# SenseTime-FVG/OpenDWM

Measured on NVIDIA H100. Metric: CTSD-3.5 6view x 16f denoise-steps/sec, higher is better.
Workload: dtype fp16

## Files before the change

opendwm_b200/csrc/common.cuh:

```cuda
#pragma once

#include <cuda.h>
#include <cuda_runtime.h>
#include <cuda_bf16.h>
#include <cuda_fp16.h>
#include <cuda_fp8.h>
#include <stdint.h>
#include <stdio.h>

namespace dwm {

void set_last_error(const char* fmt, ...);

#define DWM_CHECK_CUDA(expr)                                                   \
  do {                                                                         \
    cudaError_t _e = (expr);                                                   \
    if (_e != cudaSuccess) {                                                   \
      ::dwm::set_last_error("%s failed: %s (%s:%d)", #expr,                    \
                            cudaGetErrorString(_e), __FILE__, __LINE__);       \
      return -2;                                                               \
    }                                                                          \
  } while (0)

#define DWM_REQUIRE(cond, ...)                                                 \
  do {                                                                         \
    if (!(cond)) {                                                             \
      ::dwm::set_last_error(__VA_ARGS__);                                      \
      return -1;                                                               \
    }                                                                          \
  } while (0)

int make_tmap_2d(CUtensorMap* map, const void* base, uint64_t rows, uint64_t cols,
                 uint64_t ld, uint32_t box_rows, uint32_t box_cols, int elem_bytes);

int make_tmap_nd(CUtensorMap* map, const void* base, int rank, const uint64_t* dims,
                 const uint64_t* strides_bytes, const uint32_t* box, int elem_bytes);

int sm_count();

inline bool is_aligned(const void* p, uintptr_t bytes) { return (reinterpret_cast<uintptr_t>(p) & (bytes - 1)) == 0; }

#ifdef __CUDACC__
__device__ __forceinline__ uint32_t smem_u32(const void* p) {
  return static_cast<uint32_t>(__cvta_generic_to_shared(p));
}

__device__ __forceinline__ bool elect_one() {
  uint32_t pred = 0;
  asm volatile(
      "{\n\t"
      ".reg .pred P;\n\t"
      "elect.sync _|P, 0xffffffff;\n\t"
      "selp.u32 %0, 1, 0, P;\n\t"
      "}\n"
      : "=r"(pred));
  return pred != 0;
}

__device__ __forceinline__ void mbar_init(uint64_t* bar, uint32_t count) {
  asm volatile("mbarrier.init.shared::cta.b64 [%0], %1;" ::"r"(smem_u32(bar)), "r"(count));
}
__device__ __forceinline__ void fence_barrier_init() {
  asm volatile("fence.mbarrier_init.release.cluster;" ::: "memory");
}
__device__ __forceinline__ void fence_proxy_async() {
  asm volatile("fence.proxy.async.shared::cta;" ::: "memory");
}
__device__ __forceinline__ void mbar_expect_tx(uint64_t* bar, uint32_t bytes) {
  asm volatile("mbarrier.arrive.expect_tx.shared::cta.b64 _, [%0], %1;" ::"r"(smem_u32(bar)),
               "r"(bytes)
               : "memory");
}
__device__ __forceinline__ void mbar_arrive(uint64_t* bar) {
  asm volatile("mbarrier.arrive.shared::cta.b64 _, [%0];" ::"r"(smem_u32(bar)) : "memory");
}
__device__ __forceinline__ bool mbar_try_wait(uint64_t* bar, uint32_t parity) {
  uint32_t ok;
  asm volatile(
      "{\n\t"
      ".reg .pred P;\n\t"
      "mbarrier.try_wait.parity.shared::cta.b64 P, [%1], %2;\n\t"
      "selp.u32 %0, 1, 0, P;\n\t"
      "}\n"
      : "=r"(ok)
      : "r"(smem_u32(bar)), "r"(parity)
      : "memory");
  return ok != 0;
}
__device__ __forceinline__ void mbar_wait(uint64_t* bar, uint32_t parity) {
#ifdef DWM_BOUNDED_WAIT
  for (uint32_t it = 0; it < (1u << 26); ++it) {
    if (mbar_try_wait(bar, parity)) return;
  }
  printf("dwm_b200: mbarrier wait timed out (block %d thread %d)\n", blockIdx.x, threadIdx.x);
  __trap();
#else
  while (!mbar_try_wait(bar, parity)) {
  }
#endif
}

__device__ __forceinline__ void tma_prefetch_desc(const CUtensorMap* m) {
  asm volatile("prefetch.tensormap [%0];" ::"l"(reinterpret_cast<uint64_t>(m)) : "memory");
}
__device__ __forceinline__ void tma_load_2d(const CUtensorMap* m, uint64_t* bar, void* smem,
                                            int32_t c0, int32_t c1, uint64_t cache_hint) {
  asm volatile(
      "cp.async.bulk.tensor.2d.shared::cluster.global.mbarrier::complete_tx::bytes.L2::cache_hint"
      " [%0], [%1, {%3, %4}], [%2], %5;"
      :
      : "r"(smem_u32(smem)), "l"(reinterpret_cast<uint64_t>(m)), "r"(smem_u32(bar)), "r"(c0),
        "r"(c1), "l"(cache_hint)
      : "memory");
}
constexpr uint64_t kEvictNormal = 0x1000000000000000ull;
constexpr uint64_t kEvictFirst = 0x12F0000000000000ull;
constexpr uint64_t kEvictLast = 0x14F0000000000000ull;
__device__ __forceinline__ void tma_prefetch_2d(const CUtensorMap* m, int32_t c0, int32_t c1) {
  asm volatile("cp.async.bulk.prefetch.tensor.2d.L2.global.tile [%0, {%1, %2}];" ::"l"(
                   reinterpret_cast<uint64_t>(m)),
               "r"(c0), "r"(c1)
               : "memory");
}
__device__ __forceinline__ void tma_prefetch_5d(const CUtensorMap* m, int c0, int c1, int c2, int c3, int c4) {
  asm volatile("cp.async.bulk.prefetch.tensor.5d.L2.global.tile [%0, {%1, %2, %3, %4, %5}];" ::"l"(
                   reinterpret_cast<uint64_t>(m)),
               "r"(c0), "r"(c1), "r"(c2), "r"(c3), "r"(c4)
               : "memory");
}
__device__ __forceinline__ void tma_load_5d(const CUtensorMap* m, uint64_t* bar, void* smem, int c0,
                                            int c1, int c2, int c3, int c4, uint64_t hint) {
  asm volatile(
      "cp.async.bulk.tensor.5d.shared::cluster.global.mbarrier::complete_tx::bytes.L2::cache_hint"
      " [%0], [%1, {%3, %4, %5, %6, %7}], [%2], %8;"
      :
      : "r"(smem_u32(smem)), "l"(reinterpret_cast<uint64_t>(m)), "r"(smem_u32(bar)), "r"(c0), "r"(c1),
        "r"(c2), "r"(c3), "r"(c4), "l"(hint)
      : "memory");
}

__device__ __forceinline__ uint32_t cluster_ctarank() {
  uint32_t r;
  asm volatile("mov.u32 %0, %%cluster_ctarank;" : "=r"(r));
  return r;
}
__device__ __forceinline__ void cluster_sync_all() {
  asm volatile("barrier.cluster.arrive.release.aligned;" ::: "memory");
  asm volatile("barrier.cluster.wait.acquire.aligned;" ::: "memory");
}
__device__ __forceinline__ uint32_t mapa_u32(uint32_t smem_addr, uint32_t rank) {
  uint32_t r;
  asm volatile("mapa.shared::cluster.u32 %0, %1, %2;" : "=r"(r) : "r"(smem_addr), "r"(rank));
  return r;
}
__device__ __forceinline__ void mbar_arrive_remote(uint32_t cluster_addr) {
  asm volatile("mbarrier.arrive.shared::cluster.b64 _, [%0];" ::"r"(cluster_addr) : "memory");
}
__device__ __forceinline__ void tma_load_2d_mc(const CUtensorMap* m, uint64_t* bar, void* smem, int32_t c0,
                                               int32_t c1, uint16_t mask, uint64_t cache_hint) {
  asm volatile(
      "cp.async.bulk.tensor.2d.shared::cluster.global.mbarrier::complete_tx::bytes.multicast::cluster"
      ".L2::cache_hint [%0], [%1, {%3, %4}], [%2], %5, %6;"
      :
      : "r"(smem_u32(smem)), "l"(reinterpret_cast<uint64_t>(m)), "r"(smem_u32(bar)), "r"(c0), "r"(c1),
        "h"(mask), "l"(cache_hint)
      : "memory");
}

__device__ __forceinline__ uint64_t gmma_desc_sw128(uint32_t smem_addr) {
  uint64_t d = 0;
  d |= static_cast<uint64_t>((smem_addr & 0x3FFFF) >> 4);
  d |= static_cast<uint64_t>(1) << 16;
  d |= static_cast<uint64_t>(1024 >> 4) << 32;
  d |= static_cast<uint64_t>(1) << 62;
  return d;
}
__device__ __forceinline__ void wgmma_fence() { asm volatile("wgmma.fence.sync.aligned;" ::: "memory"); }
__device__ __forceinline__ void wgmma_commit() { asm volatile("wgmma.commit_group.sync.aligned;" ::: "memory"); }
template <int N>
__device__ __forceinline__ void wgmma_wait() {
  asm volatile("wgmma.wait_group.sync.aligned %0;" ::"n"(N) : "memory");
}
template <int N>
__device__ __forceinline__ void fence_operands(float (&d)[N]) {
#pragma unroll
  for (int i = 0; i < N; ++i) asm volatile("" : "+f"(d[i])::"memory");
}
template <int R>
__device__ __forceinline__ void setmaxnreg_inc() { asm volatile("setmaxnreg.inc.sync.aligned.u32 %0;" ::"n"(R)); }
template <int R>
__device__ __forceinline__ void setmaxnreg_dec() { asm volatile("setmaxnreg.dec.sync.aligned.u32 %0;" ::"n"(R)); }

__device__ __forceinline__ float gelu_erf(float x) {
  return 0.5f * x * (1.0f + erff(x * 0.70710678118654752440f));
}
__device__ __forceinline__ float gelu_tanh(float x) {
  const float k2 = 2.0f * 0.7978845608028654f;
  const float u2 = k2 * (x + 0.044715f * x * x * x);
  return __fdividef(x, 1.0f + __expf(-u2));
}
__device__ __forceinline__ float silu(float x) { return x / (1.0f + __expf(-x)); }

template <typename T>
struct Cvt;
template <>
struct Cvt<__nv_bfloat16> {
  __device__ static __forceinline__ uint32_t pack2(float a, float b) {
    __nv_bfloat162 v = __floats2bfloat162_rn(a, b);
    return *reinterpret_cast<uint32_t*>(&v);
  }
  __device__ static __forceinline__ float2 unpack2(uint32_t u) {
    __nv_bfloat162 v = *reinterpret_cast<__nv_bfloat162*>(&u);
    return __bfloat1622float2(v);
  }
  __device__ static __forceinline__ float to_f(__nv_bfloat16 v) { return __bfloat162float(v); }
  __device__ static __forceinline__ __nv_bfloat16 from_f(float v) { return __float2bfloat16_rn(v); }
};
template <>
struct Cvt<__half> {
  __device__ static __forceinline__ uint32_t pack2(float a, float b) {
    __half2 v = __floats2half2_rn(a, b);
// ... 34 lines not shown
```

opendwm_b200/csrc/gemm.cu:

```cuda
#include <stdlib.h>
#include <string.h>

#include "gemm_epilogue.cuh"

namespace dwm {

constexpr int STAGES = 4;
constexpr int A_STAGE_BYTES = BM * BK * 2;

template <int NT>
struct GemmCfg {
  static constexpr int kBStageBytes = NT * BK * 2;
  static constexpr int kSmemBytes =
      STAGES * (A_STAGE_BYTES + kBStageBytes) + EPI_STAGE_BYTES + 1024  + 256 ;
};

template <typename TA, typename T, int EPI, int NT, int CL>
__global__ void __launch_bounds__(GEMM_THREADS, 1)
    gemm_wgmma_kernel(const __grid_constant__ CUtensorMap tmap_a,
                      const __grid_constant__ CUtensorMap tmap_b, int M, int N, int K,
                      EpiParams p) {
  constexpr int B_STAGE_BYTES = GemmCfg<NT>::kBStageBytes;
  constexpr int BKE = BK * 2 / static_cast<int>(sizeof(TA));
  extern __shared__ uint8_t smem_raw[];
  uint8_t* smem = smem_raw + ((1024u - (smem_u32(smem_raw) & 1023u)) & 1023u);
  uint8_t* smem_a = smem;
  uint8_t* smem_b = smem + STAGES * A_STAGE_BYTES;
  float* epi_stage = reinterpret_cast<float*>(smem + STAGES * (A_STAGE_BYTES + B_STAGE_BYTES));
  uint64_t* bars = reinterpret_cast<uint64_t*>(smem + STAGES * (A_STAGE_BYTES + B_STAGE_BYTES) + EPI_STAGE_BYTES);
  uint64_t* full_bar = bars;
  uint64_t* empty_bar = bars + STAGES;

  const int warp = threadIdx.x >> 5;
  const int lane = threadIdx.x & 31;
  const int wg = threadIdx.x >> 7;
  const uint32_t rank = CL == 2 ? cluster_ctarank() : 0u;

  const int m_blocks = (M + BM - 1) / BM;
  const int n_blocks = (N + NT - 1) / NT;
  const int k_blocks = (K + BKE - 1) / BKE;
  const int num_tiles = ((m_blocks + CL - 1) / CL) * n_blocks;
  const int first = static_cast<int>(blockIdx.x) / CL, step = static_cast<int>(gridDim.x) / CL;

  if (warp == 0 && lane == 0) {
    tma_prefetch_desc(&tmap_a);
    tma_prefetch_desc(&tmap_b);
    for (int s = 0; s < STAGES; ++s) {
      mbar_init(&full_bar[s], 1);
      mbar_init(&empty_bar[s], CL * EPI_WARPS);
    }
    fence_barrier_init();
  }
  if constexpr (CL == 2) cluster_sync_all(); else __syncthreads();

  if (wg == 0) {
    setmaxnreg_dec<PRODUCER_REGS>();
    if (warp == 0 && elect_one()) {
      int stage = 0;
      uint32_t phase = 0;
      for (int tile = first; tile < num_tiles; tile += step) {
        const int m_blk = (tile / n_blocks) * CL + static_cast<int>(rank);
        const int n_blk = tile % n_blocks;
        for (int kb = 0; kb < k_blocks; ++kb) {
          mbar_wait(&empty_bar[stage], phase ^ 1);
          mbar_expect_tx(&full_bar[stage], A_STAGE_BYTES + B_STAGE_BYTES);
          tma_load_2d(&tmap_a, &full_bar[stage], smem_a + stage * A_STAGE_BYTES, kb * BKE,
                      m_blk * BM, kEvictNormal);
          if constexpr (CL == 2) {
            tma_load_2d_mc(&tmap_b, &full_bar[stage], smem_b + stage * B_STAGE_BYTES + rank * (B_STAGE_BYTES / 2),
                           kb * BKE, n_blk * NT + static_cast<int>(rank) * (NT / 2), 0x3, kEvictLast);
          } else {
            tma_load_2d(&tmap_b, &full_bar[stage], smem_b + stage * B_STAGE_BYTES, kb * BKE,
                        n_blk * NT, kEvictLast);
          }
          if (++stage == STAGES) {
            stage = 0;
            phase ^= 1;
          }
        }
      }
    }
    __syncwarp();
  } else {
    setmaxnreg_inc<CONSUMER_REGS>();
    const int cw = wg - 1;
    const int wrow = cw * 64 + (warp & 3) * 16;
    float* stg = epi_stage + (warp - 4) * 512;
    int stage = 0;
    uint32_t phase = 0;
    for (int tile = first; tile < num_tiles; tile += step) {
      const int m_blk = (tile / n_blocks) * CL + static_cast<int>(rank);
      const int n_blk = tile % n_blocks;
      const int t = threadIdx.x & 127;
      prefetch_resid_tile<EPI, NT>(p, m_blk * BM + cw * 64 + (t >> 1), M, n_blk * NT, N, t & 1);
      float acc[NT / 2];
      wg_mainloop<TA, NT, CL>(acc, smem_a, A_STAGE_BYTES, cw * 64 * 128, smem_b, B_STAGE_BYTES, full_bar,
                              empty_bar, STAGES, k_blocks, stage, phase, lane, rank ^ 1u);
      if constexpr (sizeof(TA) == 1)
        dequant_frag<NT>(acc, p.a_scale, p.w_scale, m_blk * BM + wrow, M, n_blk * NT, N, lane);
      drain_tile<T, EPI, NT>(acc, stg, m_blk * BM, wrow, M, n_blk * NT, N, p, lane);
    }
  }
  if constexpr (CL == 2) cluster_sync_all();
}

int g_resid_tma = 1;

template <typename TA, typename T, int EPI, int NT, int CL>
static int launch_gemm(const dwm_linear_args* a, cudaStream_t stream) {
  constexpr int eb = static_cast<int>(sizeof(TA));
  CUtensorMap ta, tb;
  int rc = make_tmap_2d(&ta, a->A, a->M, a->K, a->lda, BM, BK * 2 / eb, eb);
  if (rc) return rc;
  rc = make_tmap_2d(&tb, a->W, a->N, a->K, a->ldw, NT / CL, BK * 2 / eb, eb);
  if (rc) return rc;

  EpiParams p;
  fill_epi_params(p, a);
  p.resid_prefetch = g_resid_tma;

  constexpr int smem_bytes = GemmCfg<NT>::kSmemBytes;
  auto kern = gemm_wgmma_kernel<TA, T, EPI, NT, CL>;
  static bool attr_set = false;
  if (!attr_set) {
    DWM_CHECK_CUDA(cudaFuncSetAttribute(kern, cudaFuncAttributeMaxDynamicSharedMemorySize, smem_bytes));
    attr_set = true;
  }
  const long long m_blocks = (a->M + BM - 1) / BM;
  const long long n_blocks = (a->N + NT - 1) / NT;
  const long long tiles = ((m_blocks + CL - 1) / CL) * n_blocks;
  const long long slots = sm_count() / CL;
  const int grid = CL * static_cast<int>(tiles < slots ? tiles : slots);
  const int Mi = static_cast<int>(a->M), Ni = static_cast<int>(a->N), Ki = static_cast<int>(a->K);
  if constexpr (CL == 1) {
    kern<<<grid, GEMM_THREADS, smem_bytes, stream>>>(ta, tb, Mi, Ni, Ki, p);
  } else {
    DWM_CHECK_CUDA(launch_cluster2(kern, grid, GEMM_THREADS, smem_bytes, stream,
                                   ta, tb, Mi, Ni, Ki, p));
  }
  DWM_CHECK_CUDA(cudaGetLastError());
  return 0;
}

int g_gemm_bn = 0;
int g_gemm_2cta = -1;

static int pick_tile_n(const dwm_linear_args* a, int cl) {
  if (a->epilogue == DWM_EPI_GEGLU || a->epilogue == DWM_EPI_GEGLU_TANH) return 256;
  if (g_gemm_bn == 128 || g_gemm_bn == 256) return g_gemm_bn;
  const long long slots = sm_count() / cl;
  const long long m_groups = ((a->M + BM - 1) / BM + cl - 1) / cl;
  const long long t256 = m_groups * ((a->N + 255) / 256), t128 = m_groups * ((a->N + 127) / 128);
  const long long waves256 = (t256 + slots - 1) / slots, waves128 = (t128 + slots - 1) / slots;
  return waves128 * 128 * 10 < waves256 * 256 * 9 ? 128 : 256;
}

template <typename TA, typename T, int EPI, int CL>
static int launch_pick_n(const dwm_linear_args* a, cudaStream_t s) {
  if (pick_tile_n(a, CL) == 128) return launch_gemm<TA, T, EPI, 128, CL>(a, s);
  return launch_gemm<TA, T, EPI, 256, CL>(a, s);
}

template <typename TA, typename T, int CL, typename TF = T>
static int dispatch_epi(const dwm_linear_args* a, cudaStream_t s) {
  if constexpr (sizeof(TA) == 2) {
    if (a->epilogue == DWM_EPI_STORE && a->act == DWM_ACT_QUICK_GELU)
      return launch_pick_n<TA, T, EPI_STORE_QUICK_GELU, CL>(a, s);
    if (a->epilogue == DWM_EPI_GEGLU_TANH) return launch_gemm<TA, T, DWM_EPI_GEGLU_TANH, 256, CL>(a, s);
  }
  switch (a->epilogue) {
    case DWM_EPI_STORE: return launch_pick_n<TA, T, DWM_EPI_STORE, CL>(a, s);
    case DWM_EPI_GEGLU: return launch_gemm<TA, T, DWM_EPI_GEGLU, 256, CL>(a, s);
    case DWM_EPI_QKNORM: return launch_pick_n<TA, T, DWM_EPI_QKNORM, CL>(a, s);
    case DWM_EPI_RESID: return launch_pick_n<TA, TF, DWM_EPI_RESID, CL>(a, s);
    case DWM_EPI_F32: return launch_pick_n<TA, TF, DWM_EPI_F32, CL>(a, s);
    default: set_last_error("dwm_b200_linear: unknown epilogue %d", a->epilogue); return -1;
  }
}

template <int CL>
static int dispatch_e4m3(const dwm_linear_args* a, cudaStream_t s) {
  if (a->out_dtype == DWM_BF16) return dispatch_epi<__nv_fp8_e4m3, __nv_bfloat16, CL>(a, s);
  return dispatch_epi<__nv_fp8_e4m3, __half, CL, __nv_bfloat16>(a, s);
}

}

namespace dwm { int g_attn_tc = -1; extern int g_ln_staged; extern int g_conv_2cta; extern int g_conv_halo; }

extern "C" int dwm_b200_set_option(const char* name, int value) {
  using namespace dwm;
  DWM_REQUIRE(name != nullptr, "dwm_b200_set_option: null name");
  if (strcmp(name, "attn_tc") == 0) { g_attn_tc = value; return 0; }
  if (strcmp(name, "ln_staged") == 0) { g_ln_staged = value; return 0; }
  if (strcmp(name, "gemm_bn") == 0) { g_gemm_bn = value; return 0; }
  if (strcmp(name, "gemm_2cta") == 0) { g_gemm_2cta = value; return 0; }
  if (strcmp(name, "resid_tma") == 0) { g_resid_tma = value; return 0; }
  if (strcmp(name, "conv_2cta") == 0) { g_conv_2cta = value; return 0; }
  if (strcmp(name, "conv_halo") == 0) { g_conv_halo = value; return 0; }
  set_last_error("dwm_b200_set_option: unknown option %s", name);
  return -1;
}

extern "C" int dwm_b200_linear(const dwm_linear_args* a, dwm_stream_t stream) {
  using namespace dwm;
  DWM_REQUIRE(a != nullptr, "dwm_b200_linear: null args");
  DWM_REQUIRE(a->M > 0 && a->N > 0 && a->K > 0, "dwm_b200_linear: empty problem %lld x %lld x %lld",
              (long long)a->M, (long long)a->N, (long long)a->K);
  DWM_REQUIRE(a->M < (1ll << 31) && a->N < (1ll << 31) && a->K < (1ll << 31),
              "dwm_b200_linear: dimension exceeds int32");
  DWM_REQUIRE(a->A && a->W && a->out, "dwm_b200_linear: null A/W/out");
  DWM_REQUIRE(a->K % 8 == 0 && a->lda % 8 == 0 && a->ldw % 8 == 0,
              "dwm_b200_linear: K, lda, ldw must be multiples of 8 (16-byte TMA pitch); got %lld %lld %lld",
              (long long)a->K, (long long)a->lda, (long long)a->ldw);
  if (a->dtype == DWM_E4M3) {
    DWM_REQUIRE(a->K % 16 == 0 && a->lda % 16 == 0 && a->ldw % 16 == 0,
                "dwm_b200_linear: E4M3 needs K, lda, ldw multiples of 16 (16-byte TMA pitch); got %lld %lld %lld",
                (long long)a->K, (long long)a->lda, (long long)a->ldw);
    DWM_REQUIRE(a->a_scale && a->w_scale, "dwm_b200_linear: E4M3 operands need a_scale and w_scale");
    DWM_REQUIRE(a->out_dtype == DWM_BF16 || a->out_dtype == DWM_F16,
                "dwm_b200_linear: E4M3 operands need out_dtype DWM_BF16 or DWM_F16, got %d", a->out_dtype);
// ... 58 lines not shown
```

opendwm_b200/csrc/gemm_epilogue.cuh:

```cuda
#pragma once
#include "common.cuh"
#include "wgmma.cuh"
#include "../../include/dwm_b200.h"

namespace dwm {

constexpr int BM = 128;
constexpr int BK = 64;
constexpr int WG_K = 16;
constexpr int CONSUMER_WGS = 2;
constexpr int GEMM_THREADS = 128 * (1 + CONSUMER_WGS);
constexpr int EPI_WARPS = 4 * CONSUMER_WGS;
constexpr int EPI_STAGE_BYTES = EPI_WARPS * 16 * 32 * 4;
constexpr int PRODUCER_REGS = 40;
constexpr int CONSUMER_REGS = 232;
constexpr int EPI_STORE_QUICK_GELU = 16;

__device__ __forceinline__ float quick_gelu(float x) { return x / (1.0f + __expf(-1.702f * x)); }

struct EpiParams {
  void* out;
  long long ldo;
  const float* bias;
  int act;
  long long rows_per_item, out_item_stride, out_row_offset;
  const float* qw;
  const float* kw;
  long long qk_region;
  float eps;
  int norm_regions;
  const float* resid;
  long long ldr, resid_row_mod;
  const float* gate;
  long long gate_ld;
  const float* blend_x;
  long long ldx;
  const float* alpha;
  long long rows_per_batch;
  void* peer_out[8];
  int n_peers;
  int resid_prefetch;
  const float* a_scale;
  const float* w_scale;
};

__device__ __forceinline__ float apply_act(float v, int act) {
  switch (act) {
    case DWM_ACT_GELU_TANH: return gelu_tanh(v);
    case DWM_ACT_GELU_ERF: return gelu_erf(v);
    case DWM_ACT_SILU: return silu(v);
    case DWM_ACT_RELU: return fmaxf(v, 0.f);
    default: return v;
  }
}

__device__ __forceinline__ float resid_elem(float acc, float b, float g, float r) {
  return __fmaf_rn(__fadd_rn(acc, b), g, r);
}
__device__ __forceinline__ float blend_elem(float a, float a1, float x, float v) {
  return __fmaf_rn(a, x, __fmul_rn(a1, v));
}

__device__ __forceinline__ void st_global_v4(void* p, uint32_t a, uint32_t b, uint32_t c,
                                             uint32_t d) {
  asm volatile("st.global.v4.b32 [%0], {%1, %2, %3, %4};" ::"l"(p), "r"(a), "r"(b), "r"(c), "r"(d)
               : "memory");
}


template <int NA>
__device__ __forceinline__ void frag_chunk(const float (&acc)[NA], int c, float (&v)[16]) {
#pragma unroll
  for (int i = 0; i < 16; ++i) v[i] = acc[16 * c + i];
}

__device__ __forceinline__ void stage_dump(float* stg, int lane, const float (&v)[16]) {
  __syncwarp();
  const int r0 = lane >> 2, q0 = (lane & 3) >> 1, h = (lane & 1) * 2;
#pragma unroll
  for (int jj = 0; jj < 4; ++jj) {
    const int q = (2 * jj + q0) ^ r0;
    *reinterpret_cast<float2*>(stg + r0 * 32 + q * 4 + h) = make_float2(v[4 * jj], v[4 * jj + 1]);
    *reinterpret_cast<float2*>(stg + (r0 + 8) * 32 + q * 4 + h) = make_float2(v[4 * jj + 2], v[4 * jj + 3]);
  }
  __syncwarp();
}

__device__ __forceinline__ int frag_col(int lane, int jj, int e) { return 8 * jj + 2 * (lane & 3) + (e & 1); }

struct TileGeom {
  int bw;
  int rows;
  int w_lim;
  int h_lim;
  int img_w;
};

template <typename T, int EPI, int NT>
__device__ __forceinline__ void drain_tile(const float (&acc)[NT / 2], float* stg, int m_base, int row0, int M,
                                           int n_tile0, int N, const EpiParams& p, int lane,
                                           const TileGeom geom = TileGeom{0, 0, 0, 0, 0}) {
  constexpr bool kOut16 = (EPI == DWM_EPI_STORE || EPI == DWM_EPI_GEGLU || EPI == DWM_EPI_QKNORM ||
                           EPI == EPI_STORE_QUICK_GELU || EPI == DWM_EPI_GEGLU_TANH);
  const int rs = lane >> 3;
  const int c4 = lane & 7;

  int orow[4];
  int rrow[4];
  int item[4];
  float alpha[4];
  const int rpi = static_cast<int>(p.rows_per_item);
#pragma unroll
  for (int it = 0; it < 4; ++it) {
    int m;
    bool valid;
    if (geom.bw > 0) {
      const int r = row0 + it * 4 + rs;
      const int ph = r / geom.bw, pw = r - ph * geom.bw;
      valid = r < geom.rows && pw < geom.w_lim && ph < geom.h_lim;
      m = m_base + ph * geom.img_w + pw;
    } else {
      m = m_base + row0 + it * 4 + rs;
      valid = m < M;
    }
    if (valid) {
      int o = m;
      if (kOut16) {
        if (rpi > 0) o = (m / rpi) * static_cast<int>(p.out_item_stride) + (m % rpi);
        o += static_cast<int>(p.out_row_offset);
      }
      orow[it] = o;
      if (EPI == DWM_EPI_RESID) {
        item[it] = rpi > 0 ? m / rpi : 0;
        rrow[it] = p.resid_row_mod > 0 ? m % static_cast<int>(p.resid_row_mod)
                   : (p.resid_row_mod < 0 ? item[it] : m);
        alpha[it] = p.blend_x ? __ldg(p.alpha + (p.rows_per_batch > 0 ? m / static_cast<int>(p.rows_per_batch) : 0)) : 0.f;
      }
    } else {
      orow[it] = -1;
    }
  }

  auto stg4 = [&](int r) { return *reinterpret_cast<const float4*>(stg + r * 32 + ((c4 ^ (r & 7)) << 2)); };
  auto flush16 = [&](int ocol) {
#pragma unroll
    for (int it = 0; it < 4; ++it) {
      const float4 v = stg4(it * 4 + rs);
      if (orow[it] >= 0) {
        T* dst = reinterpret_cast<T*>(p.out) + static_cast<long long>(orow[it]) * p.ldo + ocol + c4 * 4;
        uint2 pk;
        pk.x = Cvt<T>::pack2(v.x, v.y);
        pk.y = Cvt<T>::pack2(v.z, v.w);
        *reinterpret_cast<uint2*>(dst) = pk;
        const long long eoff = static_cast<long long>(orow[it]) * p.ldo + ocol + c4 * 4;
        for (int q = 0; q < p.n_peers; ++q)
          *reinterpret_cast<uint2*>(reinterpret_cast<T*>(p.peer_out[q]) + eoff) = pk;
      }
    }
  };
  float4 rq[4], bq[4];
  auto prefetch32 = [&](int ocol) {
    if constexpr (EPI == DWM_EPI_RESID) {
      const int col = ocol + c4 * 4;
#pragma unroll
      for (int it = 0; it < 4; ++it) {
        rq[it] = make_float4(0.f, 0.f, 0.f, 0.f);
        bq[it] = make_float4(0.f, 0.f, 0.f, 0.f);
        if (orow[it] >= 0) {
          if (p.resid) rq[it] = *reinterpret_cast<const float4*>(p.resid + static_cast<long long>(rrow[it]) * p.ldr + col);
          if (p.blend_x) bq[it] = *reinterpret_cast<const float4*>(p.blend_x + static_cast<long long>(orow[it]) * p.ldx + col);
        }
      }
    }
  };
  auto flush32 = [&](int ocol) {
    const int col = ocol + c4 * 4;
    float4 b = make_float4(0.f, 0.f, 0.f, 0.f);
    if (EPI == DWM_EPI_RESID && p.bias) b = __ldg(reinterpret_cast<const float4*>(p.bias + col));
#pragma unroll
    for (int it = 0; it < 4; ++it) {
      float4 v = stg4(it * 4 + rs);
      if (orow[it] >= 0) {
        if (EPI == DWM_EPI_RESID) {
          float4 g = make_float4(1.f, 1.f, 1.f, 1.f);
          if (p.gate)
            g = __ldg(reinterpret_cast<const float4*>(p.gate + static_cast<long long>(item[it]) * p.gate_ld + col));
          v.x = resid_elem(v.x, b.x, g.x, rq[it].x); v.y = resid_elem(v.y, b.y, g.y, rq[it].y);
          v.z = resid_elem(v.z, b.z, g.z, rq[it].z); v.w = resid_elem(v.w, b.w, g.w, rq[it].w);
          if (p.blend_x) {
            const float a = alpha[it], a1 = 1.0f - alpha[it];
            v.x = blend_elem(a, a1, bq[it].x, v.x); v.y = blend_elem(a, a1, bq[it].y, v.y);
            v.z = blend_elem(a, a1, bq[it].z, v.z); v.w = blend_elem(a, a1, bq[it].w, v.w);
          }
        }
        *reinterpret_cast<float4*>(reinterpret_cast<float*>(p.out) + static_cast<long long>(orow[it]) * p.ldo + col) = v;
      }
    }
  };

  if constexpr (EPI == DWM_EPI_STORE || EPI == DWM_EPI_F32 || EPI == DWM_EPI_RESID || EPI == EPI_STORE_QUICK_GELU) {
#pragma unroll
    for (int c = 0; c < NT / 32; ++c) {
      const int n0 = n_tile0 + c * 32;
      if (n0 >= N) break;
      prefetch32(n0);
      float v[16];
      frag_chunk(acc, c, v);
      if (EPI != DWM_EPI_RESID) {
        if (p.bias) {
#pragma unroll
          for (int jj = 0; jj < 4; ++jj) {
            const float2 b = __ldg(reinterpret_cast<const float2*>(p.bias + n0 + frag_col(lane, jj, 0)));
            v[4 * jj] += b.x; v[4 * jj + 1] += b.y; v[4 * jj + 2] += b.x; v[4 * jj + 3] += b.y;
          }
        }
        if constexpr (EPI == EPI_STORE_QUICK_GELU) {
#pragma unroll
          for (int j = 0; j < 16; ++j) v[j] = quick_gelu(v[j]);
        } else if (p.act == DWM_ACT_GELU_TANH) {
#pragma unroll
          for (int j = 0; j < 16; ++j) v[j] = gelu_tanh(v[j]);
        } else if (p.act == DWM_ACT_SILU) {
#pragma unroll
          for (int j = 0; j < 16; ++j) v[j] = silu(v[j]);
        } else if (p.act == DWM_ACT_GELU_ERF) {
#pragma unroll
          for (int j = 0; j < 16; ++j) v[j] = gelu_erf(v[j]);
        } else if (p.act == DWM_ACT_RELU) {
#pragma unroll
          for (int j = 0; j < 16; ++j) v[j] = fmaxf(v[j], 0.f);
        }
      }
      stage_dump(stg, lane, v);
      if constexpr (EPI == DWM_EPI_STORE || EPI == EPI_STORE_QUICK_GELU) flush16(n0); else flush32(n0);
    }
  } else if constexpr (EPI == DWM_EPI_GEGLU || EPI == DWM_EPI_GEGLU_TANH) {
    static_assert(NT == 256, "GEGLU packs value / gate halves per 256-column tile");
#pragma unroll
    for (int c = 0; c < 4; ++c) {
      float a[16], g[16], v[16];
      frag_chunk(acc, c, a);
      frag_chunk(acc, c + 4, g);
      const float* bv = p.bias ? p.bias + n_tile0 + c * 32 : nullptr;
#pragma unroll
      for (int j = 0; j < 16; ++j) {
        float x = a[j], y = g[j];
        if (bv) {
          const int col = frag_col(lane, j >> 2, j);
          x += __ldg(bv + col);
          y += __ldg(bv + 128 + col);
        }
        v[j] = x * (EPI == DWM_EPI_GEGLU ? gelu_erf(y) : gelu_tanh(y));
      }
      stage_dump(stg, lane, v);
      flush16(n_tile0 / 2 + c * 32);
    }
  } else {
#pragma unroll
    for (int g = 0; g < NT / 64; ++g) {
      const int n0 = n_tile0 + g * 64;
      if (n0 >= N) break;
      float v0[16], v1[16];
      frag_chunk(acc, 2 * g, v0);
      frag_chunk(acc, 2 * g + 1, v1);
      if (p.bias) {
#pragma unroll
        for (int j = 0; j < 16; ++j) {
          const int col = frag_col(lane, j >> 2, j);
          v0[j] += __ldg(p.bias + n0 + col);
          v1[j] += __ldg(p.bias + n0 + 32 + col);
        }
      }
      const int region = n0 / static_cast<int>(p.qk_region);
      if (region < p.norm_regions) {
        const float* w = region == 0 ? p.qw : p.kw;
        float ss_lo = 0.f, ss_hi = 0.f;
#pragma unroll
        for (int j = 0; j < 16; ++j) {
          if ((j & 3) < 2) ss_lo += v0[j] * v0[j] + v1[j] * v1[j];
          else ss_hi += v0[j] * v0[j] + v1[j] * v1[j];
        }
        ss_lo += __shfl_xor_sync(0xffffffffu, ss_lo, 1);
        ss_lo += __shfl_xor_sync(0xffffffffu, ss_lo, 2);
        ss_hi += __shfl_xor_sync(0xffffffffu, ss_hi, 1);
        ss_hi += __shfl_xor_sync(0xffffffffu, ss_hi, 2);
        const float inv_lo = rsqrtf(ss_lo * (1.0f / 64.0f) + p.eps);
        const float inv_hi = rsqrtf(ss_hi * (1.0f / 64.0f) + p.eps);
#pragma unroll
        for (int j = 0; j < 16; ++j) {
          const int col = frag_col(lane, j >> 2, j);
          const float inv = (j & 3) < 2 ? inv_lo : inv_hi;
          v0[j] = v0[j] * inv * __ldg(w + col);
          v1[j] = v1[j] * inv * __ldg(w + 32 + col);
        }
      }
      stage_dump(stg, lane, v0);
      flush16(n0);
      stage_dump(stg, lane, v1);
      flush16(n0 + 32);
    }
  }
}

template <int NT>
__device__ __forceinline__ void dequant_frag(float (&acc)[NT / 2], const float* a_scale, const float* w_scale,
                                             int m0, int M, int n_tile0, int N, int lane) {
  const int r = m0 + (lane >> 2);
  const float s_lo = r < M ? __ldg(a_scale + r) : 0.f;
  const float s_hi = r + 8 < M ? __ldg(a_scale + r + 8) : 0.f;
#pragma unroll
  for (int g = 0; g < NT / 64; ++g) {
    float2 w[8];
#pragma unroll
    for (int jj = 0; jj < 8; ++jj) {
      const int col = n_tile0 + 8 * (8 * g + jj) + 2 * (lane & 3);
      w[jj] = col < N ? __ldg(reinterpret_cast<const float2*>(w_scale + col)) : make_float2(0.f, 0.f);
    }
#pragma unroll
    for (int jj = 0; jj < 8; ++jj) {
      const int j = 8 * g + jj;
      acc[4 * j + 0] = __fmul_rn(acc[4 * j + 0], __fmul_rn(s_lo, w[jj].x));
      acc[4 * j + 1] = __fmul_rn(acc[4 * j + 1], __fmul_rn(s_lo, w[jj].y));
      acc[4 * j + 2] = __fmul_rn(acc[4 * j + 2], __fmul_rn(s_hi, w[jj].x));
      acc[4 * j + 3] = __fmul_rn(acc[4 * j + 3], __fmul_rn(s_hi, w[jj].y));
    }
    asm volatile("" ::: "memory");
  }
}

template <int NT>
__device__ __forceinline__ void dequant_frag_vol(float (&acc)[NT / 2], float s, const float* w_scale,
                                                 int n_tile0, int N, int lane) {
#pragma unroll
  for (int g = 0; g < NT / 32; ++g) {
    constexpr int G = 4;
    float2 w[G];
#pragma unroll
    for (int jj = 0; jj < G; ++jj) {
      const int col = n_tile0 + 8 * (G * g + jj) + 2 * (lane & 3);
      w[jj] = col < N ? __ldg(reinterpret_cast<const float2*>(w_scale + col)) : make_float2(0.f, 0.f);
    }
#pragma unroll
    for (int jj = 0; jj < G; ++jj) {
      const int j = G * g + jj;
      const float sx = __fmul_rn(s, w[jj].x), sy = __fmul_rn(s, w[jj].y);
      acc[4 * j + 0] = __fmul_rn(acc[4 * j + 0], sx);
      acc[4 * j + 1] = __fmul_rn(acc[4 * j + 1], sy);
      acc[4 * j + 2] = __fmul_rn(acc[4 * j + 2], sx);
      acc[4 * j + 3] = __fmul_rn(acc[4 * j + 3], sy);
    }
    asm volatile("" ::: "memory");
  }
}

template <typename T, int NT, int CL = 1, int TAPS = 1>
__device__ __forceinline__ void wg_mainloop(float (&acc)[NT / 2], const uint8_t* smem_a, int a_stage_bytes,
                                            int a_row_off_bytes, const uint8_t* smem_b, int b_stage_bytes,
                                            uint64_t* full_bar, uint64_t* empty_bar, int stages, int k_iters,
                                            int& stage, uint32_t& phase, int lane, uint32_t peer = 0) {
#pragma unroll
  for (int i = 0; i < NT / 2; ++i) acc[i] = 0.f;
  fence_operands(acc);
  auto release = [&](int s) {
    mbar_arrive(&empty_bar[s]);
    if constexpr (CL == 2) mbar_arrive_remote(mapa_u32(smem_u32(&empty_bar[s]), peer));
  };
  int prev = -1;
  for (int ki = 0; ki < k_iters; ++ki) {
    mbar_wait(&full_bar[stage], phase);
    wgmma_fence();
#pragma unroll
    for (int t = 0; t < TAPS; ++t) {
      const uint64_t da = gmma_desc_sw128(smem_u32(smem_a + stage * a_stage_bytes + a_row_off_bytes + t * 128));
      const uint64_t db = gmma_desc_sw128(smem_u32(smem_b + stage * b_stage_bytes + t * NT * BK * 2));
#pragma unroll
      for (int k = 0; k < BK / WG_K; ++k) Wgmma<NT, T>::ss(acc, da + 2 * k, db + 2 * k, 1u);
    }
    wgmma_commit();
    wgmma_wait<1>();
    if (prev >= 0 && lane == 0) release(prev);
    prev = stage;
    if (++stage == stages) { stage = 0; phase ^= 1; }
  }
  wgmma_wait<0>();
  fence_operands(acc);
  if (prev >= 0 && lane == 0) release(prev);
}

template <int EPI, int NT>
__device__ __forceinline__ void prefetch_resid_tile(const EpiParams& p, int m, int M, int n_tile0,
                                                    int N, int half) {
  constexpr int half_cols = NT / 2;
  if constexpr (EPI == DWM_EPI_RESID) {
    if (!p.resid_prefetch) return;
    const int n0 = n_tile0 + half * half_cols;
    if (m < M && n0 < N) {
      const int cols = (N - n0) < half_cols ? (N - n0) : half_cols;
      const uint32_t bytes = static_cast<uint32_t>(cols) * 4u;
      if (p.resid) {
        if (p.resid_row_mod >= 0) {
          const long long rr = p.resid_row_mod > 0 ? m % static_cast<int>(p.resid_row_mod) : m;
          const float* src = p.resid + rr * p.ldr + n0;
          asm volatile("cp.async.bulk.prefetch.L2.global [%0], %1;" ::"l"(src), "r"(bytes) : "memory");
        }
      }
      if (p.blend_x) {
        const float* src = p.blend_x + static_cast<long long>(m) * p.ldx + n0;
        asm volatile("cp.async.bulk.prefetch.L2.global [%0], %1;" ::"l"(src), "r"(bytes) : "memory");
      }
    }
  }
}

template <typename... KArgs, typename... Args>
inline cudaError_t launch_cluster2(void (*kern)(KArgs...), int grid, int threads, int smem, cudaStream_t s,
                                   Args... args) {
  cudaLaunchConfig_t cfg = {};
  cfg.gridDim = dim3(grid);
  cfg.blockDim = dim3(threads);
  cfg.dynamicSmemBytes = smem;
  cfg.stream = s;
  cudaLaunchAttribute attr[1];
  attr[0].id = cudaLaunchAttributeClusterDimension;
  attr[0].val.clusterDim.x = 2;
  attr[0].val.clusterDim.y = 1;
  attr[0].val.clusterDim.z = 1;
  cfg.attrs = attr;
  cfg.numAttrs = 1;
  return cudaLaunchKernelEx(&cfg, kern, args...);
}

inline void fill_epi_params(EpiParams& p, const dwm_linear_args* a) {
  p.out = a->out;
  p.ldo = a->ldo;
  p.bias = a->bias;
  p.act = a->act;
  p.rows_per_item = a->rows_per_item;
  p.out_item_stride = a->out_item_stride;
  p.out_row_offset = a->out_row_offset;
  p.qw = a->q_norm_weight;
  p.kw = a->k_norm_weight;
  p.qk_region = a->qk_region;
  p.eps = a->eps;
  p.norm_regions = a->qk_norm_regions > 0 ? a->qk_norm_regions : 2;
  p.resid = a->resid;
  p.ldr = a->ldr;
  p.resid_row_mod = a->resid_row_mod;
  p.gate = a->gate;
  p.gate_ld = a->gate_ld;
  p.blend_x = a->blend_x;
  p.ldx = a->ldx;
  p.alpha = a->alpha;
  p.rows_per_batch = a->rows_per_batch;
  p.n_peers = a->n_peer_out;
  p.resid_prefetch = 1;
  for (int i = 0; i < 8; ++i) p.peer_out[i] = i < a->n_peer_out ? a->peer_out[i] : nullptr;
  p.a_scale = a->a_scale;
  p.w_scale = a->w_scale;
}

}
```

opendwm_b200/csrc/host.cu:

```cuda
#include <stdarg.h>
#include <string.h>

#include <mutex>
#include <unordered_map>

#include "common.cuh"
#include "../../include/dwm_b200.h"

namespace dwm {

static thread_local char g_last_error[1024] = "";

void set_last_error(const char* fmt, ...) {
  va_list ap;
  va_start(ap, fmt);
  vsnprintf(g_last_error, sizeof(g_last_error), fmt, ap);
  va_end(ap);
}

typedef CUresult (*EncodeTiledFn)(CUtensorMap*, CUtensorMapDataType, cuuint32_t, void*,
                                  const cuuint64_t*, const cuuint64_t*, const cuuint32_t*,
                                  const cuuint32_t*, CUtensorMapInterleave, CUtensorMapSwizzle,
                                  CUtensorMapL2promotion, CUtensorMapFloatOOBfill);

static EncodeTiledFn get_encode_fn() {
  static EncodeTiledFn fn = nullptr;
  static bool tried = false;
  if (!tried) {
    tried = true;
    void* p = nullptr;
    cudaDriverEntryPointQueryResult qres;
    cudaError_t e = cudaGetDriverEntryPoint("cuTensorMapEncodeTiled", &p, cudaEnableDefault, &qres);
    if (e == cudaSuccess && qres == cudaDriverEntryPointSuccess) fn = reinterpret_cast<EncodeTiledFn>(p);
  }
  return fn;
}

static int encode_tmap_2d(CUtensorMap* map, const void* base, uint64_t rows, uint64_t cols, uint64_t ld,
                          uint32_t box_rows, uint32_t box_cols, int elem_bytes);

namespace {
struct TmapKey {
  const void* base;
  uint64_t rows, cols, ld;
  uint32_t box_rows, box_cols;
  int elem;
  bool operator==(const TmapKey& o) const {
    return base == o.base && rows == o.rows && cols == o.cols && ld == o.ld && box_rows == o.box_rows &&
           box_cols == o.box_cols && elem == o.elem;
  }
};
struct TmapHash {
  size_t operator()(const TmapKey& k) const {
    uint64_t h = reinterpret_cast<uint64_t>(k.base) * 0x9E3779B97F4A7C15ull;
    h ^= (k.rows + 0x9E3779B97F4A7C15ull + (h << 6) + (h >> 2));
    h ^= (k.cols * 0xC2B2AE3D27D4EB4Full + (h << 6) + (h >> 2));
    h ^= (k.ld + (static_cast<uint64_t>(k.box_rows) << 40) + (static_cast<uint64_t>(k.box_cols) << 20) +
          static_cast<uint64_t>(k.elem) + (h << 6) + (h >> 2));
    return static_cast<size_t>(h);
  }
};
std::mutex g_tmap_mu;
std::unordered_map<TmapKey, CUtensorMap, TmapHash> g_tmap_cache;
}

int make_tmap_2d(CUtensorMap* map, const void* base, uint64_t rows, uint64_t cols, uint64_t ld,
                 uint32_t box_rows, uint32_t box_cols, int elem_bytes) {
  const TmapKey key{base, rows, cols, ld, box_rows, box_cols, elem_bytes};
  {
    std::lock_guard<std::mutex> lk(g_tmap_mu);
    auto it = g_tmap_cache.find(key);
    if (it != g_tmap_cache.end()) {
      memcpy(map, &it->second, sizeof(CUtensorMap));
      return 0;
    }
  }
  const int rc = encode_tmap_2d(map, base, rows, cols, ld, box_rows, box_cols, elem_bytes);
  if (rc) return rc;
  std::lock_guard<std::mutex> lk(g_tmap_mu);
  if (g_tmap_cache.size() > 8192) g_tmap_cache.clear();
  g_tmap_cache.emplace(key, *map);
  return 0;
}

static int encode_tmap_2d(CUtensorMap* map, const void* base, uint64_t rows, uint64_t cols, uint64_t ld,
                          uint32_t box_rows, uint32_t box_cols, int elem_bytes) {
  EncodeTiledFn fn = get_encode_fn();
  if (!fn) {
    set_last_error("cuTensorMapEncodeTiled not available (no CUDA driver / GPU?)");
    return -3;
  }
  cuuint64_t gdim[2] = {cols, rows};
  cuuint64_t gstride[1] = {ld * static_cast<uint64_t>(elem_bytes)};
  cuuint32_t box[2] = {box_cols, box_rows};
  cuuint32_t estr[2] = {1, 1};
  CUtensorMapDataType dt = elem_bytes == 2   ? CU_TENSOR_MAP_DATA_TYPE_BFLOAT16
                           : elem_bytes == 1 ? CU_TENSOR_MAP_DATA_TYPE_UINT8
                                             : CU_TENSOR_MAP_DATA_TYPE_FLOAT32;
  CUresult r = fn(map, dt, 2, const_cast<void*>(base), gdim, gstride, box, estr,
                  CU_TENSOR_MAP_INTERLEAVE_NONE, CU_TENSOR_MAP_SWIZZLE_128B,
                  CU_TENSOR_MAP_L2_PROMOTION_L2_256B, CU_TENSOR_MAP_FLOAT_OOB_FILL_NONE);
  if (r != CUDA_SUCCESS) {
    set_last_error("cuTensorMapEncodeTiled failed (CUresult %d) rows=%llu cols=%llu ld=%llu box=%ux%u",
                   (int)r, (unsigned long long)rows, (unsigned long long)cols,
                   (unsigned long long)ld, box_rows, box_cols);
    return -3;
  }
  return 0;
}

int make_tmap_nd(CUtensorMap* map, const void* base, int rank, const uint64_t* dims,
                 const uint64_t* strides_bytes, const uint32_t* box, int elem_bytes) {
  EncodeTiledFn fn = get_encode_fn();
  if (!fn) {
    set_last_error("cuTensorMapEncodeTiled not available (no CUDA driver / GPU?)");
    return -3;
  }
  cuuint64_t gdim[5];
  cuuint64_t gstride[4];
  cuuint32_t bx[5], estr[5];
  for (int i = 0; i < rank; ++i) { gdim[i] = dims[i]; bx[i] = box[i]; estr[i] = 1; }
  for (int i = 0; i + 1 < rank; ++i) gstride[i] = strides_bytes[i];
  CUtensorMapDataType dt = elem_bytes == 2   ? CU_TENSOR_MAP_DATA_TYPE_BFLOAT16
                           : elem_bytes == 1 ? CU_TENSOR_MAP_DATA_TYPE_UINT8
                                             : CU_TENSOR_MAP_DATA_TYPE_FLOAT32;
  CUresult r = fn(map, dt, static_cast<cuuint32_t>(rank), const_cast<void*>(base), gdim, gstride, bx, estr,
                  CU_TENSOR_MAP_INTERLEAVE_NONE, CU_TENSOR_MAP_SWIZZLE_128B, CU_TENSOR_MAP_L2_PROMOTION_L2_256B,
                  CU_TENSOR_MAP_FLOAT_OOB_FILL_NONE);
  if (r != CUDA_SUCCESS) {
    set_last_error("cuTensorMapEncodeTiled (rank %d) failed (CUresult %d)", rank, (int)r);
    return -3;
  }
  return 0;
}

int sm_count() {
  static int n = 0;
  if (n == 0) {
    int dev = 0;
    if (cudaGetDevice(&dev) != cudaSuccess) return 132;
    if (cudaDeviceGetAttribute(&n, cudaDevAttrMultiProcessorCount, dev) != cudaSuccess || n <= 0) n = 132;
  }
  return n;
}

}

extern "C" const char* dwm_b200_version(void) { return "dwm_b200 0.1 (sm_90a)"; }
extern "C" const char* dwm_b200_last_error(void) { return dwm::g_last_error; }
```

Before: 1.152.

## Store 16-bit GEMM epilogue outputs via stmatrix into swizzled smem and TMA bulk stores

Replaces the per-warp staged global stores in the GEMM epilogue with stmatrix writes into double-buffered 64x64 swizzled shared-memory boxes. One leader thread per warpgroup then issues a 3D TMA tensor store, synchronized with named barriers and bulk-group waits. Rows that straddle an item boundary fall back to manual vector stores. The goal is to cut global store instruction overhead and uncoalesced writes, at the cost of extra shared memory, barrier syncs and a more complex tail path.

```diff
diff --git a/opendwm_b200/csrc/common.cuh b/opendwm_b200/csrc/common.cuh
--- a/opendwm_b200/csrc/common.cuh
+++ b/opendwm_b200/csrc/common.cuh
@@ -33,6 +33,9 @@
 int make_tmap_2d(CUtensorMap* map, const void* base, uint64_t rows, uint64_t cols,
                  uint64_t ld, uint32_t box_rows, uint32_t box_cols, int elem_bytes);
 
+int make_tmap_3d(CUtensorMap* map, const void* base, uint64_t items, uint64_t rows, uint64_t cols,
+                 uint64_t ld, uint64_t item_ld, uint32_t box_rows, uint32_t box_cols, int elem_bytes);
+
 int make_tmap_nd(CUtensorMap* map, const void* base, int rank, const uint64_t* dims,
                  const uint64_t* strides_bytes, const uint32_t* box, int elem_bytes);
 
@@ -137,6 +140,24 @@
       : "r"(smem_u32(smem)), "l"(reinterpret_cast<uint64_t>(m)), "r"(smem_u32(bar)), "r"(c0), "r"(c1),
         "r"(c2), "r"(c3), "r"(c4), "l"(hint)
       : "memory");
+}
+
+__device__ __forceinline__ void tma_store_3d(const CUtensorMap* m, const void* smem, int c0, int c1, int c2) {
+  asm volatile("cp.async.bulk.tensor.3d.global.shared::cta.bulk_group [%0, {%2, %3, %4}], [%1];" ::"l"(
+                   reinterpret_cast<uint64_t>(m)),
+               "r"(smem_u32(smem)), "r"(c0), "r"(c1), "r"(c2)
+               : "memory");
+}
+__device__ __forceinline__ void bulk_commit() { asm volatile("cp.async.bulk.commit_group;" ::: "memory"); }
+__device__ __forceinline__ void bulk_wait_read_all() { asm volatile("cp.async.bulk.wait_group.read 0;" ::: "memory"); }
+__device__ __forceinline__ void bulk_wait_all() { asm volatile("cp.async.bulk.wait_group 0;" ::: "memory"); }
+__device__ __forceinline__ void named_bar_sync(int id, int n) {
+  asm volatile("bar.sync %0, %1;" ::"r"(id), "r"(n) : "memory");
+}
+__device__ __forceinline__ void stmatrix_x4(uint32_t addr, uint32_t r0, uint32_t r1, uint32_t r2, uint32_t r3) {
+  asm volatile("stmatrix.sync.aligned.m8n8.x4.shared.b16 [%0], {%1, %2, %3, %4};" ::"r"(addr), "r"(r0), "r"(r1),
+               "r"(r2), "r"(r3)
+               : "memory");
 }
 
 __device__ __forceinline__ uint32_t cluster_ctarank() {
diff --git a/opendwm_b200/csrc/gemm.cu b/opendwm_b200/csrc/gemm.cu
--- a/opendwm_b200/csrc/gemm.cu
+++ b/opendwm_b200/csrc/gemm.cu
@@ -8,17 +8,19 @@
 constexpr int STAGES = 4;
 constexpr int A_STAGE_BYTES = BM * BK * 2;
 
+static_assert(EPI_BOXES_BYTES >= EPI_STAGE_BYTES, "epilogue region");
 template <int NT>
 struct GemmCfg {
   static constexpr int kBStageBytes = NT * BK * 2;
   static constexpr int kSmemBytes =
-      STAGES * (A_STAGE_BYTES + kBStageBytes) + EPI_STAGE_BYTES + 1024  + 256 ;
+      STAGES * (A_STAGE_BYTES + kBStageBytes) + EPI_BOXES_BYTES + 1024  + 256 ;
 };
 
 template <typename TA, typename T, int EPI, int NT, int CL>
 __global__ void __launch_bounds__(GEMM_THREADS, 1)
     gemm_wgmma_kernel(const __grid_constant__ CUtensorMap tmap_a,
-                      const __grid_constant__ CUtensorMap tmap_b, int M, int N, int K,
+                      const __grid_constant__ CUtensorMap tmap_b,
+                      const __grid_constant__ CUtensorMap tmap_out, int M, int N, int K,
                       EpiParams p) {
   constexpr int B_STAGE_BYTES = GemmCfg<NT>::kBStageBytes;
   constexpr int BKE = BK * 2 / static_cast<int>(sizeof(TA));
@@ -26,8 +28,9 @@
   uint8_t* smem = smem_raw + ((1024u - (smem_u32(smem_raw) & 1023u)) & 1023u);
   uint8_t* smem_a = smem;
   uint8_t* smem_b = smem + STAGES * A_STAGE_BYTES;
-  float* epi_stage = reinterpret_cast<float*>(smem + STAGES * (A_STAGE_BYTES + B_STAGE_BYTES));
-  uint64_t* bars = reinterpret_cast<uint64_t*>(smem + STAGES * (A_STAGE_BYTES + B_STAGE_BYTES) + EPI_STAGE_BYTES);
+  uint8_t* epi_region = smem + STAGES * (A_STAGE_BYTES + B_STAGE_BYTES);
+  float* epi_stage = reinterpret_cast<float*>(epi_region);
+  uint64_t* bars = reinterpret_cast<uint64_t*>(epi_region + EPI_BOXES_BYTES);
   uint64_t* full_bar = bars;
   uint64_t* empty_bar = bars + STAGES;
 
@@ -86,6 +89,8 @@
     const int cw = wg - 1;
     const int wrow = cw * 64 + (warp & 3) * 16;
     float* stg = epi_stage + (warp - 4) * 512;
+    TmaOut tout{epi_out16(EPI) && p.tma_out, &tmap_out, epi_region + cw * 2 * EPI_BOX_BYTES, 1 + cw,
+                (threadIdx.x & 127) == 0, 0};
     int stage = 0;
     uint32_t phase = 0;
     for (int tile = first; tile < num_tiles; tile += step) {
@@ -98,8 +103,9 @@
                               empty_bar, STAGES, k_blocks, stage, phase, lane, rank ^ 1u);
       if constexpr (sizeof(TA) == 1)
         dequant_frag<NT>(acc, p.a_scale, p.w_scale, m_blk * BM + wrow, M, n_blk * NT, N, lane);
-      drain_tile<T, EPI, NT>(acc, stg, m_blk * BM, wrow, M, n_blk * NT, N, p, lane);
+      drain_tile<T, EPI, NT>(acc, stg, m_blk * BM, wrow, M, n_blk * NT, N, p, lane, TileGeom{0, 0, 0, 0, 0}, &tout);
     }
+    if (tout.on && tout.leader) bulk_wait_all();
   }
   if constexpr (CL == 2) cluster_sync_all();
 }
@@ -118,6 +124,21 @@
   EpiParams p;
   fill_epi_params(p, a);
   p.resid_prefetch = g_resid_tma;
+  CUtensorMap to = {};
+  if (epi_out16(EPI) && a->n_peer_out == 0) {
+    const long long rpi = a->rows_per_item > 0 ? a->rows_per_item : a->M;
+    const long long items = a->M / rpi;
+    const long long item_ld = (a->rows_per_item > 0 ? a->out_item_stride : a->M) * a->ldo;
+    const long long n_out = (EPI == DWM_EPI_GEGLU || EPI == DWM_EPI_GEGLU_TANH) ? a->N / 2 : a->N;
+    if (items > 0) {
+      rc = make_tmap_3d(&to, reinterpret_cast<const T*>(a->out) + a->out_row_offset * a->ldo, items, rpi, n_out,
+                        a->ldo, item_ld, 64, 64, 2);
+      if (rc) return rc;
+    }
+    p.tma_out = 1;
+    p.out_rpi = static_cast<int>(rpi);
+    p.out_items = static_cast<int>(items);
+  }
 
   constexpr int smem_bytes = GemmCfg<NT>::kSmemBytes;
   auto kern = gemm_wgmma_kernel<TA, T, EPI, NT, CL>;
@@ -133,10 +154,10 @@
   const int grid = CL * static_cast<int>(tiles < slots ? tiles : slots);
   const int Mi = static_cast<int>(a->M), Ni = static_cast<int>(a->N), Ki = static_cast<int>(a->K);
   if constexpr (CL == 1) {
-    kern<<<grid, GEMM_THREADS, smem_bytes, stream>>>(ta, tb, Mi, Ni, Ki, p);
+    kern<<<grid, GEMM_THREADS, smem_bytes, stream>>>(ta, tb, to, Mi, Ni, Ki, p);
   } else {
     DWM_CHECK_CUDA(launch_cluster2(kern, grid, GEMM_THREADS, smem_bytes, stream,
-                                   ta, tb, Mi, Ni, Ki, p));
+                                   ta, tb, to, Mi, Ni, Ki, p));
   }
   DWM_CHECK_CUDA(cudaGetLastError());
   return 0;
diff --git a/opendwm_b200/csrc/gemm_epilogue.cuh b/opendwm_b200/csrc/gemm_epilogue.cuh
--- a/opendwm_b200/csrc/gemm_epilogue.cuh
+++ b/opendwm_b200/csrc/gemm_epilogue.cuh
@@ -12,9 +12,16 @@
 constexpr int GEMM_THREADS = 128 * (1 + CONSUMER_WGS);
 constexpr int EPI_WARPS = 4 * CONSUMER_WGS;
 constexpr int EPI_STAGE_BYTES = EPI_WARPS * 16 * 32 * 4;
+constexpr int EPI_BOX_BYTES = 64 * 64 * 2;
+constexpr int EPI_BOXES_BYTES = CONSUMER_WGS * 2 * EPI_BOX_BYTES;
 constexpr int PRODUCER_REGS = 40;
 constexpr int CONSUMER_REGS = 232;
 constexpr int EPI_STORE_QUICK_GELU = 16;
+
+__host__ __device__ constexpr bool epi_out16(int epi) {
+  return epi == DWM_EPI_STORE || epi == DWM_EPI_GEGLU || epi == DWM_EPI_QKNORM || epi == EPI_STORE_QUICK_GELU ||
+         epi == DWM_EPI_GEGLU_TANH;
+}
 
 __device__ __forceinline__ float quick_gelu(float x) { return x / (1.0f + __expf(-1.702f * x)); }
 
@@ -42,6 +49,17 @@
   int resid_prefetch;
   const float* a_scale;
   const float* w_scale;
+  int tma_out;
+  int out_rpi, out_items;
+};
+
+struct TmaOut {
+  bool on;
+  const CUtensorMap* map;
+  uint8_t* bufs;
+  int bar;
+  bool leader;
+  uint32_t boxes;
 };
 
 __device__ __forceinline__ float apply_act(float v, int act) {
@@ -99,9 +117,9 @@
 template <typename T, int EPI, int NT>
 __device__ __forceinline__ void drain_tile(const float (&acc)[NT / 2], float* stg, int m_base, int row0, int M,
                                            int n_tile0, int N, const EpiParams& p, int lane,
-                                           const TileGeom geom = TileGeom{0, 0, 0, 0, 0}) {
-  constexpr bool kOut16 = (EPI == DWM_EPI_STORE || EPI == DWM_EPI_GEGLU || EPI == DWM_EPI_QKNORM ||
-                           EPI == EPI_STORE_QUICK_GELU || EPI == DWM_EPI_GEGLU_TANH);
+                                           const TileGeom geom = TileGeom{0, 0, 0, 0, 0}, TmaOut* tma = nullptr) {
+  constexpr bool kOut16 = epi_out16(EPI);
+  const bool use_tma = kOut16 && tma != nullptr && tma->on;
   const int rs = lane >> 3;
   const int c4 = lane & 7;
 
@@ -111,7 +129,7 @@
   float alpha[4];
   const int rpi = static_cast<int>(p.rows_per_item);
 #pragma unroll
-  for (int it = 0; it < 4; ++it) {
+  for (int it = 0; it < 4 && !use_tma; ++it) {
     int m;
     bool valid;
     if (geom.bw > 0) {
@@ -156,6 +174,56 @@
         for (int q = 0; q < p.n_peers; ++q)
           *reinterpret_cast<uint2*>(reinterpret_cast<T*>(p.peer_out[q]) + eoff) = pk;
       }
+    }
+  };
+  auto box_put = [&](const float (&v)[16], int ocol) {
+    const uint32_t buf = smem_u32(tma->bufs + (tma->boxes & 1) * EPI_BOX_BYTES);
+    const int i = lane >> 3;
+    const int r = (row0 & 63) + (i & 1) * 8 + (lane & 7);
+#pragma unroll
+    for (int q = 0; q < 2; ++q) {
+      const int c16 = ((ocol >> 5) & 1) * 4 + 2 * q + (i >> 1);
+      stmatrix_x4(buf + r * 128 + ((c16 ^ (r & 7)) << 4), Cvt<T>::pack2(v[8 * q], v[8 * q + 1]),
+                  Cvt<T>::pack2(v[8 * q + 2], v[8 * q + 3]), Cvt<T>::pack2(v[8 * q + 4], v[8 * q + 5]),
+                  Cvt<T>::pack2(v[8 * q + 6], v[8 * q + 7]));
+    }
+  };
+  auto box_store = [&](int ocol) {
+    fence_proxy_async();
+    if (tma->leader) bulk_wait_read_all();
+    named_bar_sync(tma->bar, 128);
+    const uint8_t* buf = tma->bufs + (tma->boxes & 1) * EPI_BOX_BYTES;
+    const int m0 = m_base + (row0 & ~63), col = ocol & ~63;
+    const int item = m0 / p.out_rpi, r = m0 - item * p.out_rpi;
+    if (tma->leader) {
+      if (item < p.out_items) tma_store_3d(tma->map, buf, col, r, item);
+      bulk_commit();
+    }
+    const int j0 = item < p.out_items ? p.out_rpi - r : 0;
+    const int j1 = M - m0 < 64 ? M - m0 : 64;
+    if (j0 < j1) {
+      const int t = ((row0 & 63) << 1) + lane;
+      const int c = t & 7;
+      const int n_out = (EPI == DWM_EPI_GEGLU || EPI == DWM_EPI_GEGLU_TANH) ? N / 2 : N;
+#pragma unroll 1
+      for (int j = j0 + (t >> 3); j < j1; j += 16) {
+        const int m = m0 + j;
+        if (col + 8 * c < n_out) {
+          const long long o = static_cast<long long>(m / p.out_rpi) * p.out_item_stride + m % p.out_rpi + p.out_row_offset;
+          *reinterpret_cast<uint4*>(reinterpret_cast<T*>(p.out) + o * p.ldo + col + 8 * c) =
+              *reinterpret_cast<const uint4*>(buf + j * 128 + ((c ^ (j & 7)) << 4));
+        }
+      }
+    }
+    ++tma->boxes;
+  };
+  auto put16 = [&](const float (&v)[16], int ocol, bool box_done) {
+    if (use_tma) {
+      box_put(v, ocol);
+      if (box_done) box_store(ocol);
+    } else {
+      stage_dump(stg, lane, v);
+      flush16(ocol);
     }
   };
   float4 rq[4], bq[4];
@@ -231,9 +299,14 @@
           for (int j = 0; j < 16; ++j) v[j] = fmaxf(v[j], 0.f);
         }
       }
-      stage_dump(stg, lane, v);
-      if constexpr (EPI == DWM_EPI_STORE || EPI == EPI_STORE_QUICK_GELU) flush16(n0); else flush32(n0);
-    }
+      if constexpr (kOut16) {
+        put16(v, n0, c & 1);
+      } else {
+        stage_dump(stg, lane, v);
+        flush32(n0);
+      }
+    }
+    if (use_tma && N - n_tile0 < NT && ((N - n_tile0) & 32)) box_store(N - 32);
   } else if constexpr (EPI == DWM_EPI_GEGLU || EPI == DWM_EPI_GEGLU_TANH) {
     static_assert(NT == 256, "GEGLU packs value / gate halves per 256-column tile");
 #pragma unroll
@@ -252,8 +325,7 @@
         }
         v[j] = x * (EPI == DWM_EPI_GEGLU ? gelu_erf(y) : gelu_tanh(y));
       }
-      stage_dump(stg, lane, v);
-      flush16(n_tile0 / 2 + c * 32);
+      put16(v, n_tile0 / 2 + c * 32, c & 1);
     }
   } else {
 #pragma unroll
@@ -294,10 +366,8 @@
           v1[j] = v1[j] * inv * __ldg(w + 32 + col);
         }
       }
-      stage_dump(stg, lane, v0);
-      flush16(n0);
-      stage_dump(stg, lane, v1);
-      flush16(n0 + 32);
+      put16(v0, n0, false);
+      put16(v1, n0 + 32, true);
     }
   }
 }
@@ -457,6 +527,8 @@
   for (int i = 0; i < 8; ++i) p.peer_out[i] = i < a->n_peer_out ? a->peer_out[i] : nullptr;
   p.a_scale = a->a_scale;
   p.w_scale = a->w_scale;
-}
-
-}
+  p.tma_out = 0;
+  p.out_rpi = p.out_items = 0;
+}
+
+}
diff --git a/opendwm_b200/csrc/host.cu b/opendwm_b200/csrc/host.cu
--- a/opendwm_b200/csrc/host.cu
+++ b/opendwm_b200/csrc/host.cu
@@ -43,11 +43,12 @@
 struct TmapKey {
   const void* base;
   uint64_t rows, cols, ld;
+  uint64_t items, item_ld;
   uint32_t box_rows, box_cols;
   int elem;
   bool operator==(const TmapKey& o) const {
-    return base == o.base && rows == o.rows && cols == o.cols && ld == o.ld && box_rows == o.box_rows &&
-           box_cols == o.box_cols && elem == o.elem;
+    return base == o.base && rows == o.rows && cols == o.cols && ld == o.ld && items == o.items &&
+           item_ld == o.item_ld && box_rows == o.box_rows && box_cols == o.box_cols && elem == o.elem;
   }
 };
 struct TmapHash {
@@ -55,6 +56,7 @@
     uint64_t h = reinterpret_cast<uint64_t>(k.base) * 0x9E3779B97F4A7C15ull;
     h ^= (k.rows + 0x9E3779B97F4A7C15ull + (h << 6) + (h >> 2));
     h ^= (k.cols * 0xC2B2AE3D27D4EB4Full + (h << 6) + (h >> 2));
+    h ^= (k.items * 0x165667B19E3779F9ull + k.item_ld + (h << 6) + (h >> 2));
     h ^= (k.ld + (static_cast<uint64_t>(k.box_rows) << 40) + (static_cast<uint64_t>(k.box_cols) << 20) +
           static_cast<uint64_t>(k.elem) + (h << 6) + (h >> 2));
     return static_cast<size_t>(h);
@@ -64,22 +66,40 @@
 std::unordered_map<TmapKey, CUtensorMap, TmapHash> g_tmap_cache;
 }
 
-int make_tmap_2d(CUtensorMap* map, const void* base, uint64_t rows, uint64_t cols, uint64_t ld,
-                 uint32_t box_rows, uint32_t box_cols, int elem_bytes) {
-  const TmapKey key{base, rows, cols, ld, box_rows, box_cols, elem_bytes};
-  {
-    std::lock_guard<std::mutex> lk(g_tmap_mu);
-    auto it = g_tmap_cache.find(key);
-    if (it != g_tmap_cache.end()) {
-      memcpy(map, &it->second, sizeof(CUtensorMap));
-      return 0;
-    }
-  }
-  const int rc = encode_tmap_2d(map, base, rows, cols, ld, box_rows, box_cols, elem_bytes);
-  if (rc) return rc;
+static bool tmap_cached(const TmapKey& key, CUtensorMap* map) {
+  std::lock_guard<std::mutex> lk(g_tmap_mu);
+  auto it = g_tmap_cache.find(key);
+  if (it == g_tmap_cache.end()) return false;
+  memcpy(map, &it->second, sizeof(CUtensorMap));
+  return true;
+}
+
+static void tmap_cache_put(const TmapKey& key, const CUtensorMap* map) {
   std::lock_guard<std::mutex> lk(g_tmap_mu);
   if (g_tmap_cache.size() > 8192) g_tmap_cache.clear();
   g_tmap_cache.emplace(key, *map);
+}
+
+int make_tmap_2d(CUtensorMap* map, const void* base, uint64_t rows, uint64_t cols, uint64_t ld,
+                 uint32_t box_rows, uint32_t box_cols, int elem_bytes) {
+  const TmapKey key{base, rows, cols, ld, 0, 0, box_rows, box_cols, elem_bytes};
+  if (tmap_cached(key, map)) return 0;
+  const int rc = encode_tmap_2d(map, base, rows, cols, ld, box_rows, box_cols, elem_bytes);
+  if (rc) return rc;
+  tmap_cache_put(key, map);
+  return 0;
+}
+
+int make_tmap_3d(CUtensorMap* map, const void* base, uint64_t items, uint64_t rows, uint64_t cols,
+                 uint64_t ld, uint64_t item_ld, uint32_t box_rows, uint32_t box_cols, int elem_bytes) {
+  const TmapKey key{base, rows, cols, ld, items, item_ld, box_rows, box_cols, elem_bytes};
+  if (tmap_cached(key, map)) return 0;
+  const uint64_t dims[3] = {cols, rows, items};
+  const uint64_t strides[2] = {ld * static_cast<uint64_t>(elem_bytes), item_ld * static_cast<uint64_t>(elem_bytes)};
+  const uint32_t box[3] = {box_cols, box_rows, 1};
+  const int rc = make_tmap_nd(map, base, 3, dims, strides, box, elem_bytes);
+  if (rc) return rc;
+  tmap_cache_put(key, map);
   return 0;
 }
 
```

After: 1.214 (median of 6 runs). 1.05x the previous value.
